# Antibas/eaQHM-analysis-and-synthesis-in-Python

Measured on AMD Instinct MI355X. Metric: analysis_frames_per_sec, higher is better.
Workload: dtype f64; 1 GPU; synth16k_60s_female_maxAdpt5; samples=960000, fs=16000, ls_frames_per_adaptation=63936, adaptations_executed=5, Kmax=59, track_bytes=906240000, parallelism=instants sharded x1 by LS cost; boundary records all-gathered per adaptation

## Files before the change

eaqhm-analysis-and-synthesis-in-python_amd/csrc/eaqhm_ls_common.h:

```cpp
#pragma once
#include "eaqhm_common.h"

namespace eaqhm {

#define PIVOT_TOL 2.5e-13

#define LS_NCLS 7
#define LS_BIG_CLASS (LS_NCLS - 1)

struct LsArgs {
  int mode;
  const double* s; long long L; double fs;
  const double* am_cur; const double* fm_cur; long long Lt; long long trk_t0; int Kmax;
  const int* frame_inst; const int* frame_c; const int* frame_wl; const double* frame_f0; const int* frame_K;
  const int* ncol; const int* cols; const unsigned char* seeded; const int* any_seed;
  int n_frames; int a_iter; double f0_stale; double f0min;
  double* records; double* raw_amp; double* raw_slope;
  double* scratch; size_t scratch_stride; int nmax; int Nmax; int Kcmax;
  int* work_counter;
  const unsigned short* zloc; const int* ztot; int zchunks;
  unsigned char* zflag;
  int* cls;
  unsigned long long* debug;
  int debug_diag;
// ... 85 lines not shown
  }
  __syncthreads();
  if (tid < 64) {
    double e = 0.0;
    for (int t = tid; t <= wl; t += 64) {
      const double sp = sig[mid + t], sm = sig[mid - t];
      e += W2[t] * ((t == 0) ? sp * sp : (sp * sp + sm * sm));
    }
#pragma unroll
    for (int o = 32; o > 0; o >>= 1) e += __shfl_xor(e, o);
    if (tid == 0) ssq[0] = e;
  }
  const int nm = 2 * n + 1;
  int NCH = 1;
  {
    int best = 0x7fffffff;
    for (int q = 1; q <= NCH_; ++q) {
      const int cost = ((nm * q + cthr - 1) / cthr) * ((wl + q - 1) / q + 4);
      if (cost < best) { best = cost; NCH = q; }
    }
  }
  const int CL = (wl + NCH - 1) / NCH;
  for (int task = tid; task < nm * NCH; task += nthr) {
    const int ch = task / nm, m = task - ch * nm;
    const int t0 = 1 + ch * CL, t1 = (t0 + CL - 1 < wl) ? (t0 + CL - 1) : wl;
    const double phi = (double)m * theta;
    double zr, zi, sr, si;
    sincos_cw((double)t0 * phi, &zi, &zr);
    sincos_cw(phi, &si, &sr);
    double a0 = 0, a1 = 0, a2 = 0, b0 = 0, b1 = 0, b2 = 0, b3 = 0;
    const bool rhs = m <= n;
    for (int t = t0; t <= t1; ++t) {
      if (t > t0 && ((t - t0) & 63) == 0) sincos_cw((double)t * phi, &zi, &zr);
      const double w2 = W2[t], tt = (double)t, w2t = w2 * tt;
      a0 = fma(w2, zr, a0);
      a1 = fma(w2t, zi, a1);
      a2 = fma(w2t * tt, zr, a2);
      if (rhs) {
        const double pa = PA[t], pb = PB[t];
        b0 = fma(pa, zr, b0);
        b1 = fma(pb, zi, b1);
        b2 = fma(tt * pb, zr, b2);
        b3 = fma(tt * pa, zi, b3);
      }
      const double nr = zr * sr - zi * si, ni = zr * si + zi * sr;
      zr = nr; zi = ni;
    }
    double* pp = part + (size_t)(ch * TZ_NQ) * TB + m;
    pp[0] = a0; pp[TB] = a1; pp[2 * TB] = a2;
    pp[3 * TB] = b0; pp[4 * TB] = b1; pp[5 * TB] = b2; pp[6 * TB] = b3;
  }
  __syncthreads();
  for (int q = tid; q < TZ_NQ * nm; q += nthr) {
    const int k = q / nm, m = q - k * nm;
    double v = 0.0;
    for (int ch = 0; ch < NCH; ++ch) v += part[(size_t)(ch * TZ_NQ + k) * TB + m];
    if (k < 3) v *= 2.0;
    if (k == 0) v += W2[0];
    if (k == 3 && m <= n) v += W2[0] * sig[mid];
    tab[k * TB + m] = v;
  }
  __syncthreads();
}

__device__ inline int toeplitz_harm(int c, int n) { return (c < n) ? -(c + 1) : (c - n); }
__device__ inline void toeplitz_gram(const double* tab, int TB, int p, int a, int b, int n, double& re, double& im) {
  const int m = toeplitz_harm(b, n) - toeplitz_harm(a, n), am = (m < 0) ? -m : m;
  re = 0.0; im = 0.0;
  if (p == 1) im = (m < 0) ? -tab[TB + am] : tab[TB + am];
  else re = tab[p * TB + am];
}
__device__ inline void toeplitz_rhs(const double* tab, int TB, int p, int b, int n, double& re, double& im) {
  const int h = toeplitz_harm(b, n), ah = (h < 0) ? -h : h;
  re = tab[(3 + 2 * p) * TB + ah];
  im = tab[(4 + 2 * p) * TB + ah];
  if (h < 0) im = -im;
}

#define XCOL(cc, el) (((cc) & ~15) | (((cc) + (el)) & 15))

template <int STRIDE, int NWAVES>
__device__ inline void prepare_slots(const LsArgs& A, double* Qf, double* Af, int Npad, double* ci,
                                     unsigned long long* masks, int* gappy, const int* mycols, int n, int N, int mid,
                                     int c, int wl, bool seeds, int lane, int wave, int nchs) {
  const double eps = 10e-5;
  const int nch = (N + 63) >> 6;
  const long long t0 = (long long)c - wl;
  const unsigned short* zloc = uni(A.zloc);
  const int* ztot = uni(A.ztot);
  const double* fm_all = uni(A.fm_cur);
  const double* am_all = uni(A.am_cur);
  const long long L = ((long long)uni((int)(A.Lt >> 32)) << 32) | (unsigned)uni((int)(A.Lt & 0xffffffffll));
  const int zchunks = uni(A.zchunks);
  const double w1 = uni(2.0 * M_PI / A.fs);
  auto centre = [&](int j, double fv, double av) {
    ci[j * STRIDE + STRIDE - 3] = 1.0 / (av + eps);
    double sn, cs;
    sincos_cw(fv * w1, &sn, &cs);
    ci[j * STRIDE + STRIDE - 2] = cs;
    ci[j * STRIDE + STRIDE - 1] = sn;
  };
  int anyg = 0;
  for (int j = threadIdx.x; j < n; j += blockDim.x) {
    const int k = mycols[j];
    const long long b = (long long)c + wl, a1 = (long long)c - wl - 1;
    const int cb = (int)(b >> 10), ca = (a1 >= 0) ? (int)(a1 >> 10) : 0;
    const double fmc = fm_all[(size_t)k * L + c], amc = am_all[(size_t)k * L + c];
    int zc = zloc[(size_t)k * L + b];
    for (int ch = ca; ch < cb; ++ch) zc += ztot[(size_t)k * zchunks + ch];
    if (a1 >= 0) zc -= zloc[(size_t)k * L + a1];
    const int g = (zc != 0 || (seeds && k == 0)) ? 1 : 0;
    gappy[j] = g;
    anyg |= g;
    ci[j * STRIDE + 0] = 0.0;
    ci[j * STRIDE + 1] = 0.0;
    const size_t trk = (size_t)k * L + t0;
    ((const double**)(ci + j * STRIDE))[2] = g ? (Qf + (size_t)j * Npad) : (fm_all + trk);
    ((const double**)(ci + j * STRIDE))[3] = g ? (Af + (size_t)j * Npad) : (am_all + trk);
    if (!g) centre(j, fmc, amc);
  }
  if (!__syncthreads_or(anyg)) return;
  for (int it = wave; it < n * nch; it += NWAVES) {
    const int j = it / nch, ch = it - j * nch, t = (ch << 6) + lane;
    if (!gappy[j]) continue;
    const double fv = (t < N) ? track_fm(A, mycols[j], t0 + t, c, seeds) : 0.0;
    const unsigned long long m = __ballot(fv != 0.0);
    if (lane == 0) masks[j * nchs + ch] = m;
  }
  __syncthreads();
  for (int it = wave; it < n * nch; it += NWAVES) {
    const int j = it / nch, ch = it - j * nch, t = (ch << 6) + lane, k = mycols[j];
    if (!gappy[j] || t >= N) continue;
    double fv = track_fm(A, k, t0 + t, c, seeds), av = track_am(A, k, t0 + t, c, seeds);
    if (fv == 0.0) {
      int p = -1, q = -1;
      {
        unsigned long long m = masks[j * nchs + ch] & ((lane == 0) ? 0ull : (~0ull >> (64 - lane)));
        int cc = ch;
        while (m == 0ull && cc > 0) { --cc; m = masks[j * nchs + cc]; }
        if (m != 0ull) p = (cc << 6) + 63 - __clzll((long long)m);
      }
      {
        unsigned long long m = masks[j * nchs + ch] & ((lane == 63) ? 0ull : (~0ull << (lane + 1)));
        int cc = ch;
        while (m == 0ull && cc < nch - 1) { ++cc; m = masks[j * nchs + cc]; }
        if (m != 0ull) q = (cc << 6) + __ffsll((long long)m) - 1;
      }
      if (p < 0) {
        fv = track_fm(A, k, t0 + q, c, seeds); av = track_am(A, k, t0 + q, c, seeds);
      } else if (q < 0) {
        fv = track_fm(A, k, t0 + p, c, seeds); av = track_am(A, k, t0 + p, c, seeds);
      } else {
        const double f0v = track_fm(A, k, t0 + p, c, seeds), f1v = track_fm(A, k, t0 + q, c, seeds);
        const double a0v = track_am(A, k, t0 + p, c, seeds), a1v = track_am(A, k, t0 + q, c, seeds);
        const double dx = (double)(q - p), xx = (double)(t - p);
        fv = ((f1v - f0v) / dx) * xx + f0v;
        av = ((a1v - a0v) / dx) * xx + a0v;
      }
    }
    Qf[(size_t)j * Npad + t] = fv;
    Af[(size_t)j * Npad + t] = av;
    if (t == mid) centre(j, fv, av);
  }
  __syncthreads();
}

template <int CTRL>
__device__ inline double dpp_row(double x) {
  const int lo = __builtin_amdgcn_update_dpp(0, __double2loint(x), CTRL, 0xf, 0xf, true);
  const int hi = __builtin_amdgcn_update_dpp(0, __double2hiint(x), CTRL, 0xf, 0xf, true);
  return __hiloint2double(hi, lo);
}
__device__ inline double scan16(double x) {
  x += dpp_row<0x111>(x);
  x += dpp_row<0x112>(x);
  x += dpp_row<0x114>(x);
  x += dpp_row<0x118>(x);
  return x;
}

__device__ inline void cholesky_solve(double* __restrict__ Lt, int M, int ldl, double* rowj, double* xs, double* sh,
                                      int* fault) {
  const int tid = threadIdx.x, nt = blockDim.x;
  for (int j = 0; j < M; ++j) {
    for (int k = tid; k < j; k += nt) {
      size_t o = ((size_t)k * ldl + j) * 2;
      rowj[2 * k] = Lt[o];
      rowj[2 * k + 1] = Lt[o + 1];
    }
    __syncthreads();
    for (int i = j + tid; i <= M; i += nt) {
      size_t oj = ((size_t)j * ldl + i) * 2;
      double ar = Lt[oj], ai = Lt[oj + 1];
      for (int k = 0; k < j; ++k) {
        size_t o = ((size_t)k * ldl + i) * 2;
        double lr = Lt[o], li = Lt[o + 1];
        double cr = rowj[2 * k], ci = rowj[2 * k + 1];
        ar -= lr * cr + li * ci;
        ai -= li * cr - lr * ci;
      }
      if (i == j) {
        if (!(ar > PIVOT_TOL * Lt[oj])) { atomicAdd(fault, 1); ar = 1.0; }
        double d = sqrt(ar);
        sh[0] = d;
        Lt[oj] = d; Lt[oj + 1] = 0.0;
      } else {
        Lt[oj] = ar; Lt[oj + 1] = ai;
      }
    }
    __syncthreads();
    double inv = 1.0 / sh[0];
    for (int i = j + 1 + tid; i <= M; i += nt) {
      size_t oj = ((size_t)j * ldl + i) * 2;
      Lt[oj] *= inv; Lt[oj + 1] *= inv;
    }
    __syncthreads();
  }
  if (tid < 64) {
    for (int j = M - 1; j >= 0; --j) {
      const double* row = Lt + (size_t)j * ldl * 2;
      double sr = 0, si = 0;
      for (int i = j + 1 + tid; i < M; i += 64) {
        double lr = row[2 * i], li = row[2 * i + 1];
        double xr = xs[2 * i], xi = xs[2 * i + 1];
        sr += lr * xr + li * xi;
        si += lr * xi - li * xr;
      }
      for (int o = 32; o > 0; o >>= 1) {
        sr += __shfl_xor(sr, o);
        si += __shfl_xor(si, o);
      }
      if (tid == 0) {
        double d = row[2 * j];
        double yr = row[2 * M], yi = -row[2 * M + 1];
        xs[2 * j] = (yr - sr) / d;
        xs[2 * j + 1] = (yi - si) / d;
      }
      __builtin_amdgcn_wave_barrier();
      __threadfence_block();
    }
  }
  __syncthreads();
}

__device__ inline void write_record(const LsArgs& A, const double* xs, double* sh, const int* mycols, int f, int n,
                                    int inst, int c, double f0, bool seeds) {
  const int tid = threadIdx.x, nt = blockDim.x, Kc = 2 * n + 1;
  if (A.raw_amp) {
    const int stride = 2 * (2 * A.Kmax + 1);
    for (int q = tid; q < 2 * Kc; q += nt) {
      const int col = q >> 1, src = (A.mode == 0 && col < n) ? (n - 1 - col) : col;
      A.raw_amp[(size_t)f * stride + q] = xs[2 * src + (q & 1)];
      A.raw_slope[(size_t)f * stride + q] = xs[2 * Kc + 2 * src + (q & 1)];
    }
  }
  double amax = 0.0;
  for (int j = tid; j < n; j += nt) {
    double ar = xs[2 * (n + 1 + j)], ai = xs[2 * (n + 1 + j) + 1];
    amax = fmax(amax, sqrt(ar * ar + ai * ai));
  }
  for (int o = 32; o > 0; o >>= 1) amax = fmax(amax, __shfl_xor(amax, o));
  if ((tid & 63) == 0) sh[1 + (tid >> 6)] = amax;
  __syncthreads();
  amax = 0.0;
  for (int w = 0; w < (nt >> 6); ++w) amax = fmax(amax, sh[1 + w]);
  const double floor_mag = amax * 3.1622776601683795e-08;
  const double h = f0 / (double)(A.a_iter + 1);
  double* rec = A.records + (size_t)inst * (3 * A.Kmax + 1);
  for (int k = tid; k < 3 * A.Kmax; k += nt) rec[k] = 0.0;
  __syncthreads();
  for (int j = tid; j < n; j += nt) {
    const int k = (A.mode == 0) ? j : mycols[j];
    double ar = xs[2 * (n + 1 + j)], ai = xs[2 * (n + 1 + j) + 1];
    double br = xs[2 * (Kc + n + 1 + j)], bi = xs[2 * (Kc + n + 1 + j) + 1];
    double mag = sqrt(ar * ar + ai * ai);
    double eta = 0.0;
    if (A.mode == 1) eta = A.fs / (2.0 * M_PI) * ((ar * bi - ai * br) / (mag * mag));
    if (mag > floor_mag && fabs(eta) < h) {
      rec[k] = mag;
      rec[2 * A.Kmax + k] = atan2(ai, ar);
      double fmv;
      if (A.mode == 0) fmv = (double)(k + 1) * f0;
      else {
        double cur = track_fm(A, k, c, c, seeds);
        fmv = (f0 > A.f0min) ? cur + eta : cur;
      }
      rec[A.Kmax + k] = fmv;
    }
  }
  if (tid == 0) rec[3 * A.Kmax] = xs[2 * n];
  __syncthreads();
}

}
```

eaqhm-analysis-and-synthesis-in-python_amd/csrc/eaqhm_ls_tile.hip:

```cpp
#include <type_traits>
#include "eaqhm_ls_common.h"
#include "eaqhm_ls_chol.h"
#include "eaqhm_ls_a0.h"
#include "eaqhm_ls_tilemap.h"
#include "eaqhm_ls_twunits.h"
#include "eaqhm_ls_gather.h"

namespace eaqhm {
bool ls_a0tile_fits(const LsArgs& A);
int launch_ls_a0tile(eaqhm_ctx* ctx, LsArgs A);

#define DIAG_OWNER(jb, nt) ((int)TL_DIAG[nt][jb])
#define TL_THREADS 512
#define TL_WAVES 8
#define TL_CW 8
#define TL_NTMAX 13
#define CI_STRIDE 20
#define CI_NCH 16

__device__ inline void tw_step(d4 (&g)[9], double aR, double aI, double bR, double bI, double nk) {
  const double sA = aR + aI, dB = bI - bR;
  const double naR = nk * aR, naI = nk * aI, nsA = nk * sA;
  const double nbR = nk * bR, nbI = nk * bI, ndB = nk * dB;
  g[0] = __builtin_amdgcn_mfma_f64_16x16x4f64(aR, bR, g[0], 0, 0, 0);
  g[1] = __builtin_amdgcn_mfma_f64_16x16x4f64(aI, bI, g[1], 0, 0, 0);
  g[2] = __builtin_amdgcn_mfma_f64_16x16x4f64(sA, dB, g[2], 0, 0, 0);
  g[3] = __builtin_amdgcn_mfma_f64_16x16x4f64(naR, bR, g[3], 0, 0, 0);
  g[4] = __builtin_amdgcn_mfma_f64_16x16x4f64(naI, bI, g[4], 0, 0, 0);
  g[5] = __builtin_amdgcn_mfma_f64_16x16x4f64(nsA, dB, g[5], 0, 0, 0);
  g[6] = __builtin_amdgcn_mfma_f64_16x16x4f64(naR, nbR, g[6], 0, 0, 0);
  g[7] = __builtin_amdgcn_mfma_f64_16x16x4f64(naI, nbI, g[7], 0, 0, 0);
  g[8] = __builtin_amdgcn_mfma_f64_16x16x4f64(nsA, ndB, g[8], 0, 0, 0);
}

__device__ inline void twu_pair_k3(d4 (&g0)[3], d4 (&g1)[3], d4 (&g2)[3], double aR, double aI, double bR, double bI, double nk) {
  const double sA = aR + aI, dB = bI - bR;
  const double naR = nk * aR, naI = nk * aI, nsA = nk * sA;
  const double nbR = nk * bR, nbI = nk * bI, ndB = nk * dB;
  g0[0] = __builtin_amdgcn_mfma_f64_16x16x4f64(aR, bR, g0[0], 0, 0, 0);
  g0[1] = __builtin_amdgcn_mfma_f64_16x16x4f64(aI, bI, g0[1], 0, 0, 0);
  g0[2] = __builtin_amdgcn_mfma_f64_16x16x4f64(sA, dB, g0[2], 0, 0, 0);
  g1[0] = __builtin_amdgcn_mfma_f64_16x16x4f64(naR, bR, g1[0], 0, 0, 0);
  g1[1] = __builtin_amdgcn_mfma_f64_16x16x4f64(naI, bI, g1[1], 0, 0, 0);
  g1[2] = __builtin_amdgcn_mfma_f64_16x16x4f64(nsA, dB, g1[2], 0, 0, 0);
  g2[0] = __builtin_amdgcn_mfma_f64_16x16x4f64(naR, nbR, g2[0], 0, 0, 0);
  g2[1] = __builtin_amdgcn_mfma_f64_16x16x4f64(naI, nbI, g2[1], 0, 0, 0);
  g2[2] = __builtin_amdgcn_mfma_f64_16x16x4f64(nsA, ndB, g2[2], 0, 0, 0);
}
__device__ inline void twu_pair_2acc(d4 (&g0)[2], d4 (&g1)[2], d4 (&g2)[2], double aR, double aI, double bR, double bI, double nk,
                                     bool k4) {
  const double naR = nk * aR, naI = nk * aI, nbR = nk * bR, nbI = nk * bI;
  g0[0] = __builtin_amdgcn_mfma_f64_16x16x4f64(aR, bR, g0[0], 0, 0, 0);
  g1[0] = __builtin_amdgcn_mfma_f64_16x16x4f64(naR, bR, g1[0], 0, 0, 0);
  g2[0] = __builtin_amdgcn_mfma_f64_16x16x4f64(naR, nbR, g2[0], 0, 0, 0);
  g0[1] = __builtin_amdgcn_mfma_f64_16x16x4f64(aR, bI, g0[1], 0, 0, 0);
  g1[1] = __builtin_amdgcn_mfma_f64_16x16x4f64(naR, bI, g1[1], 0, 0, 0);
  g2[1] = __builtin_amdgcn_mfma_f64_16x16x4f64(naR, nbI, g2[1], 0, 0, 0);
  g0[0] = __builtin_amdgcn_mfma_f64_16x16x4f64(aI, bI, g0[0], 0, 0, 0);
  g1[0] = __builtin_amdgcn_mfma_f64_16x16x4f64(naI, bI, g1[0], 0, 0, 0);
  g2[0] = __builtin_amdgcn_mfma_f64_16x16x4f64(naI, nbI, g2[0], 0, 0, 0);
  if (k4) {
    const double maI = -aI, mnaI = -naI;
    g0[1] = __builtin_amdgcn_mfma_f64_16x16x4f64(maI, bR, g0[1], 0, 0, 0);
    g1[1] = __builtin_amdgcn_mfma_f64_16x16x4f64(mnaI, bR, g1[1], 0, 0, 0);
    g2[1] = __builtin_amdgcn_mfma_f64_16x16x4f64(mnaI, nbR, g2[1], 0, 0, 0);
  }
}

__device__ inline void twu_edge_k4(d4 (&g0)[2], d4 (&g1)[2], double aR, double aI, double bR, double bI, double nk) {
  const double nbR = nk * bR, nbI = nk * bI, maI = -aI;
  g0[0] = __builtin_amdgcn_mfma_f64_16x16x4f64(aR, bR, g0[0], 0, 0, 0);
  g1[0] = __builtin_amdgcn_mfma_f64_16x16x4f64(aR, nbR, g1[0], 0, 0, 0);
  g0[1] = __builtin_amdgcn_mfma_f64_16x16x4f64(aR, bI, g0[1], 0, 0, 0);
  g1[1] = __builtin_amdgcn_mfma_f64_16x16x4f64(aR, nbI, g1[1], 0, 0, 0);
  g0[0] = __builtin_amdgcn_mfma_f64_16x16x4f64(aI, bI, g0[0], 0, 0, 0);
  g1[0] = __builtin_amdgcn_mfma_f64_16x16x4f64(aI, nbI, g1[0], 0, 0, 0);
  g0[1] = __builtin_amdgcn_mfma_f64_16x16x4f64(maI, bR, g0[1], 0, 0, 0);
  g1[1] = __builtin_amdgcn_mfma_f64_16x16x4f64(maI, nbR, g1[1], 0, 0, 0);
}

template <int NS, int TW, int UA = 0, int UB = 0, int TB = 0>
__device__ __attribute__((noinline)) void tile_frame(const LsArgs& A, int TS_, int ldx_max_, double* lds, int f_) {
  const int TS = uni(TS_), ldx_max = uni(ldx_max_), f = uni(f_);
  const int tid = threadIdx.x, nt_thr = TL_THREADS;
  const int lane = tid & 63;
  const int wave = __builtin_amdgcn_readfirstlane(tid >> 6);
  double* U = uni(lds);
  double* Xre = U;
  double* Xim = Xre + (size_t)TS * ldx_max;
  const size_t usize_g = (size_t)2 * TS * ldx_max;
  double* ci = U + usize_g;
  unsigned long long* masks = (unsigned long long*)(ci + (size_t)CI_STRIDE * 52);
  double* PanR = U;
  double* PanI = PanR + TL_NTMAX * TL_TILE;
  double* WtR = PanI + TL_NTMAX * TL_TILE;
  double* WtI = WtR + TL_NTMAX * TL_TILE;
  double* LdR = WtI + TL_NTMAX * TL_TILE;
  double* LdI = LdR + TL_TILE;
  double* Dc = LdI + TL_TILE;
  double* Zc = Dc + DG_TILE;
  double* zv = Zc + DG_TILE;
  double* xv = zv + 2 * 16 * TL_NTMAX;
  const size_t usize_c = (size_t)(xv + 32 - U);
  double* xs = U + usize_c;
  double* sh = xs + 4 * uni(A.Kcmax);
  double* win = sh + 16;
  double* sig = win + 64 * CI_NCH;
  double* dorig = sig + 64 * CI_NCH;

  const int Npad = ((uni(A.Nmax) + 63) >> 6) << 6;
  double* Qs = uni(A.scratch) + (size_t)blockIdx.x * (size_t)uni((int)A.scratch_stride);
  double* Rs = Qs + (size_t)Npad * uni(A.nmax);
  const bool seeds = uni((int)(A.any_seed && (*A.any_seed != 0))) != 0;
  const double w1 = uni(2.0 * M_PI / A.fs);
  const int PE = TS / 2;
  const double* sA = uni(A.s);
  const int lcol = lane & 15, lq = lane >> 4;
  unsigned long long* dbg = uni(A.debug);
  unsigned long long t_prev = 0;

  {
    const int n = uni(A.ncol[f]);
    const int Kc = 2 * n + 1, Ms = 2 * Kc + 1;
    const int nt = (Ms + 15) >> 4;
    const int c = uni(A.frame_c[f]), wl = uni(A.frame_wl[f]), inst = uni(A.frame_inst[f]);
    const int N = 2 * wl + 1, mid = wl;
    const int T = (Kc + 16) >> 4;
    constexpr int UN = UA + UB;
    constexpr int GA = UA / 3, GB = UB / 3;
    constexpr bool G3 = TW > 0 || UN > 0;
    static_assert(TW == 0 || UN == 0, "whole pairs or units");
    static_assert(UN == 0 || (UA == TWU_UA && UB == TWU_UB), "slot layout of eaqhm_ls_twunits.h");
    static_assert(TB >= 0 && TB < TWU_NTB, "unit table");
    constexpr bool PK = UN > 0 && TWU_PACKED[TB];
    constexpr int EC = 16 * (TWU_TT[TB] - 1);
    const int nb = G3 ? T : nt;
    const int ldx = (nb << 4) + ((nb & 1) ? 0 : 16);
    const int npair = T * (T + 1) / 2;
    const int is = 2 * Kc - 16 * (nt - 1);
    const double f0 = uni(A.f0_stale);
    const int* mycols = uni(A.cols) + (size_t)f * uni(A.Kmax);
    const int npairs = mid + 1;

    if (dbg && tid == 0) t_prev = __builtin_amdgcn_s_memtime();
    for (int q = tid; q < 2 * TS * ldx_max; q += nt_thr) Xre[q] = 0.0;
    for (int t = tid; t < N; t += nt_thr) {
      win[t] = window_value(false, t, N);
      sig[t] = sA[(size_t)(c - wl) + t];
    }
    __syncthreads();
    int* gappy = (int*)(masks + (size_t)52 * CI_NCH);
    prepare_slots<CI_STRIDE, TL_WAVES>(A, Qs, Rs, Npad, ci, masks, gappy, mycols, n, N, mid, c, wl, seeds, lane, wave, CI_NCH);
    LS_STAMP(0);

    constexpr int NM3 = (NS <= 7) ? NS : 0;
    d4 accR[NS], accI[NS], acc3[NM3 ? NM3 : 1];
    int tP[NS], tQ[NS];
    bool live[NS];
#pragma unroll
    for (int sl = 0; sl < NS; ++sl) {
      accR[sl] = (d4){0, 0, 0, 0};
      accI[sl] = (d4){0, 0, 0, 0};
      if (sl < NM3) acc3[sl] = (d4){0, 0, 0, 0};
      const int code = TL_MAP[nt][wave][sl];
      live[sl] = code != 0xFF;
      const int P = live[sl] ? (code >> 4) : 0, Q = live[sl] ? (code & 15) : 0;
      tP[sl] = __builtin_amdgcn_readfirstlane(P);
      tQ[sl] = __builtin_amdgcn_readfirstlane(Q);
    }

    constexpr int TWA = TW ? TW : 1;
    const bool split = TW > 0 && NS == 5 && T == 4;
    d4 g[TWA][9];
    int gI[TWA], gJ[TWA], gx[TWA];
    bool glive[TWA];
#pragma unroll
    for (int sl = 0; sl < TWA; ++sl) {
      const int x = (split && sl == 1) ? 8 + (wave >> 1) : wave + 8 * sl;
      glive[sl] = TW && x < npair && !(split && sl == 1 && wave >= 4);
      gx[sl] = __builtin_amdgcn_readfirstlane(x);
      int I = 0, J = 0;
      if (glive[sl]) tile_of(x, I, J);
      gI[sl] = __builtin_amdgcn_readfirstlane(I);
      gJ[sl] = __builtin_amdgcn_readfirstlane(J);
#pragma unroll
      for (int p = 0; p < 9; ++p) g[sl][p] = (d4){0, 0, 0, 0};
    }

    constexpr int UAA = UA > 3 ? UA : 3, UBA = UB > 3 ? UB : 3;
    d4 ga[UAA][3], gb[UBA][2];
    int ucode[UN ? UN : 1];
    if constexpr (UN > 0) {
#pragma unroll
      for (int sl = 0; sl < UN; ++sl) ucode[sl] = __builtin_amdgcn_readfirstlane((int)TWU_MAPS[TB][wave][sl]);
#pragma unroll
      for (int sl = 0; sl < UA; ++sl)
#pragma unroll
        for (int p = 0; p < 3; ++p) ga[sl][p] = (d4){0, 0, 0, 0};
#pragma unroll
      for (int sl = 0; sl < UB; ++sl) gb[sl][0] = gb[sl][1] = (d4){0, 0, 0, 0};
    }

    for (int d0 = 0; d0 < npairs; d0 += PE) {
#pragma clang loop unroll(disable)
      for (int idx = tid; idx < 16 * n; idx += nt_thr) {
        const int el = idx & 15, j = idx >> 4, d = d0 + el;
        const bool act = d <= mid;
        const int u = mid - d - 1, v = mid + d;
        double su = 0, cu = 1, sv, cv;
        double pur = 0, pui = 0, nur = 0, nui = 0, pvr, pvi, nvr, nvi;
        {
          double* cj = ci + j * CI_STRIDE;
          const double* fb = ((const double**)cj)[2];
          const double* ab = ((const double**)cj)[3];
          const int dc = act ? d : mid;
          const double fu1 = fb[mid - dc], fv = fb[mid + dc];
          const double au = ab[(mid - dc - 1 >= 0) ? (mid - dc - 1) : 0], au1 = ab[mid - dc];
          const double av = ab[mid + dc], av1 = ab[(mid + dc + 1 < N) ? (mid + dc + 1) : (N - 1)];
          const double xu = act ? fu1 : 0.0, xv = (act && d >= 1) ? fv : 0.0;
          const double qv = cj[0] + scan16(xv), qu = -(cj[1] + scan16(xu));
          if (el == 15) { cj[0] = qv; cj[1] = -qu; }
          if (!act) continue;
          const double ainv = cj[17], pr = cj[18], pi = cj[19];
          sincos_cw(qu * w1, &su, &cu);
          sincos_cw(qv * w1, &sv, &cv);
          const double eps = 10e-5;
          if (u >= 0) {
            const double ru = (eps + au) * ainv, rv1 = (eps + av1) * ainv;
            pur = ru * cu;                    pui = ru * su;
            nur = rv1 * (cv * pr - sv * pi);  nui = rv1 * (cv * pi + sv * pr);
          }
          const double rv = (eps + av) * ainv, ru1 = (eps + au1) * ainv;
          pvr = rv * cv;                      pvi = rv * sv;
          nvr = ru1 * (cu * pr - su * pi);    nvi = ru1 * (cu * pi + su * pr);
        }
// ... 359 lines not shown
      }
      LS_STAMP(uni((int)A.debug_diag) ? 2 : 9);
    }

    {
#pragma unroll
      for (int sl = 0; sl < NS; ++sl) {
        if (!live[sl] || tP[sl] != nt - 1) continue;
#pragma unroll
        for (int r = 0; r < 4; ++r) {
          const int row = lq + 4 * r, col = lcol;
          const bool pad = (row > is) || (tQ[sl] == nt - 1 && col > is);
          if (pad) {
            accR[sl][r] = (tQ[sl] == nt - 1 && row == col) ? 1.0 : 0.0;
            accI[sl][r] = 0.0;
          }
        }
      }
#pragma unroll
      for (int sl = 0; sl < NS; ++sl) {
        if (!live[sl] || tP[sl] != tQ[sl]) continue;
#pragma unroll
        for (int r = 0; r < 4; ++r)
          if (lq + 4 * r == lcol) dorig[16 * tP[sl] + lcol] = accR[sl][r];
      }
      double* post = Dc;
      double* dumpD = Dc + DGP_DOUBLES;
      double* zs = dumpD + 128;
      int* dflag = (int*)(zs + 256);
      if (tid == 0) *dflag = 0;
      __syncthreads();
#define TRAILING_UPDATE(sl)                                                                         \
  {                                                                                                 \
    const double* ar = PanR + tP[sl] * TL_TILE;                                                     \
    const double* ai = PanI + tP[sl] * TL_TILE;                                                     \
    const double* br = PanR + tQ[sl] * TL_TILE;                                                     \
    const double* bi = PanI + tQ[sl] * TL_TILE;                                                     \
       \
       \
    d4 p1 = (d4){0, 0, 0, 0}, p2 = (d4){0, 0, 0, 0};                                                \
    _Pragma("unroll") for (int ks = 0; ks < 4; ++ks) {                                              \
      const int o = (4 * ks + lq) * TL_LD + lcol;                                                   \
      const double aR = ar[o], aI = ai[o], lR = br[o], lI = bi[o];                                  \
      p1 = __builtin_amdgcn_mfma_f64_16x16x4f64(aR, lR, p1, 0, 0, 0);                               \
      p2 = __builtin_amdgcn_mfma_f64_16x16x4f64(aI, lI, p2, 0, 0, 0);                               \
      accI[sl] = __builtin_amdgcn_mfma_f64_16x16x4f64(aR + aI, lI - lR, accI[sl], 0, 0, 0);         \
    }                                                                                               \
    accR[sl] = accR[sl] - (p1 + p2);                                                                \
    accI[sl] = accI[sl] + (p1 - p2);                                                                \
  }
      for (int jb = 0; jb < nt; ++jb) {
        d4 Rt = (d4){0, 0, 0, 0}, It = (d4){0, 0, 0, 0};
        bool mine = false;
#pragma unroll
        for (int sl = 0; sl < NS; ++sl) {
          if (!live[sl] || tP[sl] != jb || tQ[sl] != jb) continue;
          if (jb > 0) TRAILING_UPDATE(sl)
          Rt = accR[sl]; It = accI[sl];
          mine = true;
        }
        if (mine) {
          unsigned long long td0 = 0;
          unsigned long long* tlast = (unsigned long long*)(dflag + 2);
          const bool tdiag = dbg && uni(A.debug_diag);
          if (tdiag) td0 = __builtin_amdgcn_s_memtime();
          diag_D(Rt, It, post, nullptr, dflag, 16 * jb, dumpD, LdR, LdI, jb == nt - 1);
          if (tdiag && lane == 0) {
            const unsigned long long td1 = __builtin_amdgcn_s_memtime();
            atomicAdd(dbg + 9, td1 - td0);
            if (jb > 0) { atomicAdd(dbg + 11, td0 - *tlast); atomicAdd(dbg + 14, 1ull); }
            atomicAdd(dbg + 13, 1ull);
            *tlast = td1;
          }
        }
        LS_STAMP(10);
        if (jb > 0) {
#pragma unroll
          for (int sl = 0; sl < NS; ++sl) {
            if (!live[sl] || tQ[sl] < jb || (tP[sl] == jb && tQ[sl] == jb)) continue;
            TRAILING_UPDATE(sl)
          }
        }
        LS_STAMP(8);
        if (!mine && wave == (int)TL_HELP[nt][jb])
          diag_Z(post, dflag, 16 * jb, zs, WtR + jb * TL_TILE, WtI + jb * TL_TILE, dorig + 16 * jb,
                 (jb == nt - 1) ? is : 16, uni(A.fault));
        __syncthreads();
        LS_STAMP(6);
#pragma unroll
        for (int sl = 0; sl < NS; ++sl) {
          if (!live[sl] || tQ[sl] != jb || tP[sl] == jb) continue;
          double* tr = PanR + tP[sl] * TL_TILE;
          double* ti = PanI + tP[sl] * TL_TILE;
#pragma unroll
          for (int r = 0; r < 4; ++r) {
            tr[lcol * TL_LD + lq + 4 * r] = accR[sl][r];
            ti[lcol * TL_LD + lq + 4 * r] = accI[sl][r];
          }
          __builtin_amdgcn_wave_barrier();
          d4 p1 = (d4){0, 0, 0, 0}, p2 = (d4){0, 0, 0, 0}, p3 = (d4){0, 0, 0, 0};
          const double* wr = WtR + jb * TL_TILE;
          const double* wi = WtI + jb * TL_TILE;
#pragma unroll
          for (int ks = 0; ks < 4; ++ks) {
            const int o = (4 * ks + lq) * TL_LD + lcol;
            const double aR = tr[o], aI = ti[o], bR = wr[o], bI = wi[o];
            p1 = __builtin_amdgcn_mfma_f64_16x16x4f64(aR, bR, p1, 0, 0, 0);
            p2 = __builtin_amdgcn_mfma_f64_16x16x4f64(aI, bI, p2, 0, 0, 0);
            p3 = __builtin_amdgcn_mfma_f64_16x16x4f64(aR + aI, bR + bI, p3, 0, 0, 0);
          }
          const d4 xr = p1 - p2, xi = p3 - (p1 + p2);
          accR[sl] = xr; accI[sl] = xi;
          __builtin_amdgcn_wave_barrier();
#pragma unroll
          for (int r = 0; r < 4; ++r) {
            tr[lcol * TL_LD + lq + 4 * r] = xr[r];
            ti[lcol * TL_LD + lq + 4 * r] = xi[r];
          }
        }
        LS_STAMP(7);
        __syncthreads();
      }
#undef TRAILING_UPDATE
      __syncthreads();
      LS_STAMP(3);

#pragma unroll
      for (int sl = 0; sl < NS; ++sl) {
        if (!live[sl] || tP[sl] != nt - 1 || tQ[sl] == nt - 1) continue;
        if (lq == (is & 3)) {
#pragma unroll
          for (int r = 0; r < 4; ++r)
            if (r == (is >> 2)) {
              zv[2 * (16 * tQ[sl] + lcol)] = accR[sl][r];
              zv[2 * (16 * tQ[sl] + lcol) + 1] = -accI[sl][r];
            }
        }
      }
      if (tid < 16) {
        const bool ok = tid < is;
        zv[2 * (16 * (nt - 1) + tid)] = ok ? LdR[is * TL_LD + tid] : 0.0;
        zv[2 * (16 * (nt - 1) + tid) + 1] = ok ? -LdI[is * TL_LD + tid] : 0.0;
      }
      for (int q = tid; q < 4 * Kc; q += nt_thr) xs[q] = 0.0;
      __syncthreads();
      for (int P = nt - 1; P >= 0; --P) {
        if (tid < 256) {
          const int i = tid >> 4, k = tid & 15;
          double xr = 0, xi = 0;
          if (k >= i) {
            const double wr = WtR[P * TL_TILE + i * TL_LD + k], wi = WtI[P * TL_TILE + i * TL_LD + k];
            const double zr = zv[2 * (16 * P + k)], zi = zv[2 * (16 * P + k) + 1];
            xr = wr * zr - wi * zi;
            xi = wr * zi + wi * zr;
          }
#pragma unroll
          for (int o = 8; o > 0; o >>= 1) { xr += __shfl_xor(xr, o); xi += __shfl_xor(xi, o); }
          if (k == 0) {
            xv[2 * i] = xr; xv[2 * i + 1] = xi;
            const int q = 16 * P + i;
            if (q < 2 * Kc) { xs[2 * q] = xr; xs[2 * q + 1] = xi; }
          }
        }
        __syncthreads();
#pragma unroll
        for (int sl = 0; sl < NS; ++sl) {
          if (!live[sl] || tP[sl] != P || tQ[sl] == P) continue;
          double sr = 0, si = 0;
#pragma unroll
          for (int r = 0; r < 4; ++r) {
            const double xr = xv[2 * (lq + 4 * r)], xi = xv[2 * (lq + 4 * r) + 1];
            const double lr = accR[sl][r], li = accI[sl][r];
            sr += lr * xr + li * xi;
            si += lr * xi - li * xr;
          }
          sr += __shfl_xor(sr, 16); si += __shfl_xor(si, 16);
          sr += __shfl_xor(sr, 32); si += __shfl_xor(si, 32);
          if (lq == 0) {
            zv[2 * (16 * tQ[sl] + lcol)] -= sr;
            zv[2 * (16 * tQ[sl] + lcol) + 1] -= si;
          }
        }
        __syncthreads();
      }
      LS_STAMP(4);
    }

    write_record(A, xs, sh, mycols, f, n, inst, c, f0, seeds);
    LS_STAMP(5);
  }
}

__device__ inline int frame_class(int n) {
  const int nt = (2 * (2 * n + 1) + 1 + 15) >> 4;
  return nt <= 8 ? 0 : nt == 9 ? 1 : nt == 10 ? 2 : nt == 11 ? 3 : nt == 12 ? 4 : nt <= TL_NTMAX ? 5 : LS_BIG_CLASS;
}
extern "C" __global__ void __launch_bounds__(256) eaqhm_ls_classify_kernel(LsArgs A) {
  const int f = blockIdx.x * blockDim.x + threadIdx.x, lane = threadIdx.x & 63;
  int cl = (f < A.n_frames) ? frame_class((A.mode == 0) ? A.frame_K[f] : A.ncol[f]) : -1;
  if (f < A.n_frames) {
    if (!frame_window_ok(A, A.frame_c[f], A.frame_wl[f])) { cl = -1; atomicAdd(A.fault + 2, 1); }
  }
  if (A.mode == 1 && cl >= 0) {
    const long long c = A.frame_c[f], wl = A.frame_wl[f];
    const long long lo = (c - wl - 1 > 0) ? (c - wl - 1) : 0;
    for (long long ch = lo >> 10; ch <= ((c + wl) >> 10); ++ch) A.zflag[ch] = 1;
  }
  for (int c = 0; c < LS_NCLS; ++c) {
    const unsigned long long m = __ballot(cl == c);
    if (m == 0ull) continue;
    int base = 0;
    if (lane == __ffsll((long long)m) - 1) base = atomicAdd(A.cls + c, __popcll(m));
    base = __shfl(base, __ffsll((long long)m) - 1);
    if (cl == c) A.cls[16 + (size_t)c * A.n_frames + base + __popcll(m & ((1ull << lane) - 1ull))] = f;
  }
}

extern "C" __global__ void __launch_bounds__(256) eaqhm_ls_zero_prefix_kernel(const double* __restrict__ fm, long long Lt,
                                                                              long long t_lo, int ch0, int zchunks,
                                                                              const unsigned char* __restrict__ zflag,
                                                                              unsigned short* __restrict__ zloc,
                                                                              int* __restrict__ ztot) {
  __shared__ int wsum[4];
  const int k = blockIdx.y, ch = ch0 + blockIdx.x, tid = threadIdx.x, lane = tid & 63, wave = tid >> 6;
  if (!zflag[ch]) return;
  const long long base = (long long)ch << 10;
  int run = 0;
  for (int p = 0; p < 4; ++p) {
    const long long t = base + 256 * p + tid;
    const bool in = t >= t_lo && t < t_lo + Lt;
    const bool z = in && (fm[(size_t)k * Lt + t] == 0.0);
    const unsigned long long m = __ballot(z);
    const int incl = __popcll(m & ((lane == 63) ? ~0ull : ((1ull << (lane + 1)) - 1ull)));
    if (lane == 0) wsum[wave] = __popcll(m);
    __syncthreads();
    int off = 0, tot = 0;
#pragma unroll
    for (int w = 0; w < 4; ++w) { const int v = wsum[w]; tot += v; if (w < wave) off += v; }
    if (in) zloc[(size_t)k * Lt + t] = (unsigned short)(run + off + incl);
    run += tot;
    __syncthreads();
  }
  if (tid == 0) ztot[(size_t)k * zchunks + ch] = run;
}

extern "C" __global__ void __launch_bounds__(TL_THREADS) eaqhm_ls_tile_kernel(LsArgs A, int TS, int ldx_max) {
  extern __shared__ __attribute__((aligned(16))) double lds[];
  __shared__ int nxt;
#define TW_UNITS(TB) 0, TWU_UA, TWU_UB, TB
#define RUN_CLASS(NSV, TWV, C)                                                             \
  for (;;) {                                                                             \
    if (threadIdx.x == 0) nxt = atomicAdd(A.cls + 8 + C, 1);                             \
    __syncthreads();                                                                     \
    const int item = nxt;                                                                \
    __syncthreads();                                                                     \
    if (item >= A.cls[C]) break;                                                         \
    if (A.mode == 0) a0_frame<A0_NS, A0_M, 2>(A, lds, A.cls[16 + (size_t)C * A.n_frames + item], TZ_TB, TZ_NCH, 520, 64 * CI_NCH);                          \
    else tile_frame<NSV, TWV>(A, TS, ldx_max, lds, A.cls[16 + (size_t)C * A.n_frames + item]);          \
  }
  RUN_CLASS(12, 0, 5)
  RUN_CLASS(10, TW_UNITS(TWU_TB_12), 4)
  RUN_CLASS(9, TW_UNITS(TWU_TB_11), 3)
  RUN_CLASS(7, 2, 2)
  RUN_CLASS(6, 2, 1)
  RUN_CLASS(5, 2, 0)
#undef RUN_CLASS
#undef TW_UNITS
}

#define TL_LDS_LIMIT (159 * 1024)
static size_t tl_usize_c() {
  return (size_t)4 * TL_NTMAX * TL_TILE + 2 * TL_TILE + 2 * DG_TILE + 2 * 16 * TL_NTMAX + 32;
}
static size_t tl_usize_g(int TS, int ldx_max) { return (size_t)2 * TS * ldx_max + (size_t)CI_STRIDE * 52 + 52 * CI_NCH + 32; }
static size_t tl_lds_doubles(int Kcmax, int TS, int ldx_max) {
  const size_t c = tl_usize_c(), g = tl_usize_g(TS, ldx_max);
  return (c > g ? c : g) + 4 * (size_t)Kcmax + 16 + 2 * 64 * CI_NCH + 16 * TL_NTMAX;
}

bool ls_tile_applicable(int Kcmax, int Nmax) {
  return Nmax <= 64 * CI_NCH && tl_lds_doubles(Kcmax, 32, 16 * TL_NTMAX + 16) * sizeof(double) <= TL_LDS_LIMIT;
}

size_t ls_tile_scratch_stride(int nmax, int Nmax) {
  const size_t Npad = (size_t)((Nmax + 63) >> 6) << 6;
  const size_t bridged = 2 * Npad * nmax, gram = (size_t)3 * 21 * 512 + 2;
  return ((bridged > gram ? bridged : gram) + 15) & ~(size_t)15;
}

int launch_ls_prepass(eaqhm_ctx* ctx, LsArgs A, long long track_t0) {
  hipLaunchKernelGGL(eaqhm_ls_classify_kernel, dim3((A.n_frames + 255) / 256), dim3(256), 0, ctx->stream, A);
  HIP_TRY(ctx, hipGetLastError());
  if (A.mode == 1) {
    const int ch0 = (int)(track_t0 >> 10), ch1 = (int)((track_t0 + A.Lt - 1) >> 10);
    hipLaunchKernelGGL(eaqhm_ls_zero_prefix_kernel, dim3(ch1 - ch0 + 1, A.Kmax), dim3(256), 0, ctx->stream, A.fm_cur, A.Lt,
                       track_t0, ch0, A.zchunks, A.zflag, (unsigned short*)A.zloc, (int*)A.ztot);
    HIP_TRY(ctx, hipGetLastError());
  }
  return EAQHM_OK;
}

int launch_ls_tile(eaqhm_ctx* ctx, LsArgs A, int grid) {
  if (A.mode == 0 && ctx->a0_resident && ls_a0tile_fits(A)) return launch_ls_a0tile(ctx, A);
  const int Kcmax = A.Kcmax;
  const int ldx_max = 16 * TL_NTMAX + 16;
  const int TS = 32;
  const size_t lds_bytes = tl_lds_doubles(Kcmax, TS, ldx_max) * sizeof(double);
  if (lds_bytes > TL_LDS_LIMIT) return ctx->fail(EAQHM_EINVAL, "eaqhm_ls_batch: LDS budget exceeded (tile variant)");
  if (a0_lds_doubles(A0_M, 2, TZ_TB, TZ_NCH, 520, 64 * CI_NCH, Kcmax) * sizeof(double) > lds_bytes)
    return ctx->fail(EAQHM_EINVAL, "eaqhm_ls_batch: LDS budget exceeded (adaptation 0, tile variant)");
  HIP_TRY(ctx, hipFuncSetAttribute((const void*)eaqhm_ls_tile_kernel, hipFuncAttributeMaxDynamicSharedMemorySize, (int)lds_bytes));
  hipLaunchKernelGGL(eaqhm_ls_tile_kernel, dim3(grid), dim3(TL_THREADS), lds_bytes, ctx->stream, A, TS, ldx_max);
  HIP_TRY(ctx, hipGetLastError());
  return EAQHM_OK;
}

}
```

Before: 1.659 million frames/s.

## Prefetch next frame header during solve and stage records in LDS

Adds a persistent LDS header so one idle wave fetches the next work item (atomic, frame params, column list) during the Cholesky phase, removing the serialized atomic plus barriers between frames. Also replaces shuffle reductions with DPP/permlane-swap reductions, overlaps signal loads with zeroing of the X tiles, and for the NS=9 class builds the output record in LDS with a cached centre frequency before copying it out contiguously. This adds LDS layout constraints, more control complexity and a new header region whose placement must not overlap other buffers.

```diff
diff --git a/eaqhm-analysis-and-synthesis-in-python_amd/csrc/eaqhm_ls_common.h b/eaqhm-analysis-and-synthesis-in-python_amd/csrc/eaqhm_ls_common.h
--- a/eaqhm-analysis-and-synthesis-in-python_amd/csrc/eaqhm_ls_common.h
+++ b/eaqhm-analysis-and-synthesis-in-python_amd/csrc/eaqhm_ls_common.h
@@ -191,7 +191,7 @@
 template <int STRIDE, int NWAVES>
 __device__ inline void prepare_slots(const LsArgs& A, double* Qf, double* Af, int Npad, double* ci,
                                      unsigned long long* masks, int* gappy, const int* mycols, int n, int N, int mid,
-                                     int c, int wl, bool seeds, int lane, int wave, int nchs) {
+                                     int c, int wl, bool seeds, int lane, int wave, int nchs, double* fstash = nullptr) {
   const double eps = 10e-5;
   const int nch = (N + 63) >> 6;
   const long long t0 = (long long)c - wl;
@@ -227,6 +227,7 @@
     ((const double**)(ci + j * STRIDE))[2] = g ? (Qf + (size_t)j * Npad) : (fm_all + trk);
     ((const double**)(ci + j * STRIDE))[3] = g ? (Af + (size_t)j * Npad) : (am_all + trk);
     if (!g) centre(j, fmc, amc);
+    if (fstash) fstash[j] = g ? -1.0 : fmc;
   }
   if (!__syncthreads_or(anyg)) return;
   for (int it = wave; it < n * nch; it += NWAVES) {
@@ -287,6 +288,32 @@
   x += dpp_row<0x118>(x);
   return x;
 }
+__device__ inline double sum16_first(double x) {
+  x += dpp_row<0x108>(x);
+  x += dpp_row<0x104>(x);
+  x += dpp_row<0x102>(x);
+  x += dpp_row<0x101>(x);
+  return x;
+}
+__device__ inline double sum4rows_first(double x) {
+  {
+    const auto lo = __builtin_amdgcn_permlane16_swap(__double2loint(x), __double2loint(x), false, false);
+    const auto hi = __builtin_amdgcn_permlane16_swap(__double2hiint(x), __double2hiint(x), false, false);
+    x = __hiloint2double(hi[0], lo[0]) + __hiloint2double(hi[1], lo[1]);
+  }
+  const auto lo = __builtin_amdgcn_permlane32_swap(__double2loint(x), __double2loint(x), false, false);
+  const auto hi = __builtin_amdgcn_permlane32_swap(__double2hiint(x), __double2hiint(x), false, false);
+  return __hiloint2double(hi[0], lo[0]) + __hiloint2double(hi[1], lo[1]);
+}
+__device__ inline double max64_nonneg_last(double x) {
+  x = fmax(x, dpp_row<0x111>(x));
+  x = fmax(x, dpp_row<0x112>(x));
+  x = fmax(x, dpp_row<0x114>(x));
+  x = fmax(x, dpp_row<0x118>(x));
+  x = fmax(x, dpp_row<0x142>(x));
+  x = fmax(x, dpp_row<0x143>(x));
+  return x;
+}
 
 __device__ inline void cholesky_solve(double* __restrict__ Lt, int M, int ldl, double* rowj, double* xs, double* sh,
                                       int* fault) {
@@ -352,8 +379,10 @@
   __syncthreads();
 }
 
+template <bool ROW = false>
 __device__ inline void write_record(const LsArgs& A, const double* xs, double* sh, const int* mycols, int f, int n,
-                                    int inst, int c, double f0, bool seeds) {
+                                    int inst, int c, double f0, bool seeds, const double* fstash = nullptr,
+                                    double* row = nullptr) {
   const int tid = threadIdx.x, nt = blockDim.x, Kc = 2 * n + 1;
   if (A.raw_amp) {
     const int stride = 2 * (2 * A.Kmax + 1);
@@ -368,16 +397,25 @@
     double ar = xs[2 * (n + 1 + j)], ai = xs[2 * (n + 1 + j) + 1];
     amax = fmax(amax, sqrt(ar * ar + ai * ai));
   }
-  for (int o = 32; o > 0; o >>= 1) amax = fmax(amax, __shfl_xor(amax, o));
-  if ((tid & 63) == 0) sh[1 + (tid >> 6)] = amax;
+  if constexpr (ROW) {
+    amax = max64_nonneg_last(amax);
+    if ((tid & 63) == 63) sh[1 + (tid >> 6)] = amax;
+    for (int k = tid; k < 3 * A.Kmax; k += nt) row[k] = 0.0;
+  } else {
+    for (int o = 32; o > 0; o >>= 1) amax = fmax(amax, __shfl_xor(amax, o));
+    if ((tid & 63) == 0) sh[1 + (tid >> 6)] = amax;
+  }
   __syncthreads();
   amax = 0.0;
   for (int w = 0; w < (nt >> 6); ++w) amax = fmax(amax, sh[1 + w]);
   const double floor_mag = amax * 3.1622776601683795e-08;
   const double h = f0 / (double)(A.a_iter + 1);
   double* rec = A.records + (size_t)inst * (3 * A.Kmax + 1);
-  for (int k = tid; k < 3 * A.Kmax; k += nt) rec[k] = 0.0;
-  __syncthreads();
+  double* dst = ROW ? row : rec;
+  if constexpr (!ROW) {
+    for (int k = tid; k < 3 * A.Kmax; k += nt) rec[k] = 0.0;
+    __syncthreads();
+  }
   for (int j = tid; j < n; j += nt) {
     const int k = (A.mode == 0) ? j : mycols[j];
     double ar = xs[2 * (n + 1 + j)], ai = xs[2 * (n + 1 + j) + 1];
@@ -386,19 +424,21 @@
     double eta = 0.0;
     if (A.mode == 1) eta = A.fs / (2.0 * M_PI) * ((ar * bi - ai * br) / (mag * mag));
     if (mag > floor_mag && fabs(eta) < h) {
-      rec[k] = mag;
-      rec[2 * A.Kmax + k] = atan2(ai, ar);
+      dst[k] = mag;
+      dst[2 * A.Kmax + k] = atan2(ai, ar);
       double fmv;
       if (A.mode == 0) fmv = (double)(k + 1) * f0;
       else {
-        double cur = track_fm(A, k, c, c, seeds);
+        double cur = (ROW && fstash[j] >= 0.0) ? fstash[j] : track_fm(A, k, c, c, seeds);
         fmv = (f0 > A.f0min) ? cur + eta : cur;
       }
-      rec[A.Kmax + k] = fmv;
-    }
-  }
-  if (tid == 0) rec[3 * A.Kmax] = xs[2 * n];
-  __syncthreads();
-}
-
-}
+      dst[A.Kmax + k] = fmv;
+    }
+  }
+  if (tid == 0) dst[3 * A.Kmax] = xs[2 * n];
+  __syncthreads();
+  if constexpr (ROW)
+    for (int k = tid; k <= 3 * A.Kmax; k += nt) rec[k] = row[k];
+}
+
+}
diff --git a/eaqhm-analysis-and-synthesis-in-python_amd/csrc/eaqhm_ls_tile.hip b/eaqhm-analysis-and-synthesis-in-python_amd/csrc/eaqhm_ls_tile.hip
--- a/eaqhm-analysis-and-synthesis-in-python_amd/csrc/eaqhm_ls_tile.hip
+++ b/eaqhm-analysis-and-synthesis-in-python_amd/csrc/eaqhm_ls_tile.hip
@@ -5,6 +5,7 @@
 #include "eaqhm_ls_tilemap.h"
 #include "eaqhm_ls_twunits.h"
 #include "eaqhm_ls_gather.h"
+#include "eaqhm_ls_tilelds.h"
 
 namespace eaqhm {
 bool ls_a0tile_fits(const LsArgs& A);
@@ -14,9 +15,23 @@
 #define TL_THREADS 512
 #define TL_WAVES 8
 #define TL_CW 8
-#define TL_NTMAX 13
-#define CI_STRIDE 20
-#define CI_NCH 16
+static_assert(TLL_TILE == TL_TILE && TLL_DG_TILE == DG_TILE, "eaqhm_ls_tilelds.h and eaqhm_ls_chol.h disagree");
+
+__device__ inline void fetch_next_header(const LsArgs& A, TlHead* hd, int C, int nbuf, int lane) {
+  int* cls = uni(A.cls);
+  int item = 0;
+  if (lane == 0) item = atomicAdd(cls + 8 + C, 1);
+  item = uni(item);
+  int f = -1;
+  if (item < uni(cls[C])) f = uni(cls[16 + (size_t)C * uni(A.n_frames) + item]);
+  if (f >= 0) {
+    const int* tab = (lane == 0) ? A.ncol : (lane == 1) ? A.frame_c : (lane == 2) ? A.frame_wl : A.frame_inst;
+    if (lane < 4) (&hd->n)[lane] = tab[f];
+    const int Kmax = uni(A.Kmax);
+    if (lane < TL_NSLOT && lane < Kmax) hd->cols[nbuf][lane] = A.cols[(size_t)f * Kmax + lane];
+  }
+  if (lane == 0) { hd->f = f; hd->buf = nbuf; hd->cls = C; }
+}
 
 __device__ inline void tw_step(d4 (&g)[9], double aR, double aI, double bR, double bI, double nk) {
   const double sA = aR + aI, dB = bI - bR;
@@ -81,11 +96,17 @@
 
 template <int NS, int TW, int UA = 0, int UB = 0, int TB = 0>
 __device__ __attribute__((noinline)) void tile_frame(const LsArgs& A, int TS_, int ldx_max_, double* lds, int f_) {
-  const int TS = uni(TS_), ldx_max = uni(ldx_max_), f = uni(f_);
+  constexpr int C = NS == 12 ? 5 : NS == 10 ? 4 : NS == 9 ? 3 : NS == 7 ? 2 : NS == 6 ? 1 : 0;
+  static_assert(NS == 12 || NS == 10 || NS == 9 || NS == 7 || NS == 6 || NS == 5, "a register budget per class");
+  constexpr bool NEXT_HEAD = NS != 10, REC_ROW = NS == 9;
+  const bool pre = uni(f_) < 0;
+  const int TS = uni(TS_), ldx_max = uni(ldx_max_);
   const int tid = threadIdx.x, nt_thr = TL_THREADS;
   const int lane = tid & 63;
   const int wave = __builtin_amdgcn_readfirstlane(tid >> 6);
   double* U = uni(lds);
+  TlHead* hd = (TlHead*)(U + tl_head_offset());
+  const int f = pre ? uni(hd->f) : uni(f_);
   double* Xre = U;
   double* Xim = Xre + (size_t)TS * ldx_max;
   const size_t usize_g = (size_t)2 * TS * ldx_max;
@@ -101,8 +122,7 @@
   double* Zc = Dc + DG_TILE;
   double* zv = Zc + DG_TILE;
   double* xv = zv + 2 * 16 * TL_NTMAX;
-  const size_t usize_c = (size_t)(xv + 32 - U);
-  double* xs = U + usize_c;
+  double* xs = xv + 32 + TL_HEAD_DOUBLES;
   double* sh = xs + 4 * uni(A.Kcmax);
   double* win = sh + 16;
   double* sig = win + 64 * CI_NCH;
@@ -111,7 +131,7 @@
   const int Npad = ((uni(A.Nmax) + 63) >> 6) << 6;
   double* Qs = uni(A.scratch) + (size_t)blockIdx.x * (size_t)uni((int)A.scratch_stride);
   double* Rs = Qs + (size_t)Npad * uni(A.nmax);
-  const bool seeds = uni((int)(A.any_seed && (*A.any_seed != 0))) != 0;
+  const bool seeds = uni(hd->seeds) != 0;
   const double w1 = uni(2.0 * M_PI / A.fs);
   const int PE = TS / 2;
   const double* sA = uni(A.s);
@@ -120,10 +140,11 @@
   unsigned long long t_prev = 0;
 
   {
-    const int n = uni(A.ncol[f]);
+    const int n = pre ? uni(hd->n) : uni(A.ncol[f]);
     const int Kc = 2 * n + 1, Ms = 2 * Kc + 1;
     const int nt = (Ms + 15) >> 4;
-    const int c = uni(A.frame_c[f]), wl = uni(A.frame_wl[f]), inst = uni(A.frame_inst[f]);
+    const int c = pre ? uni(hd->c) : uni(A.frame_c[f]), wl = pre ? uni(hd->wl) : uni(A.frame_wl[f]);
+    const int inst = pre ? uni(hd->inst) : uni(A.frame_inst[f]);
     const int N = 2 * wl + 1, mid = wl;
     const int T = (Kc + 16) >> 4;
     constexpr int UN = UA + UB;
@@ -139,18 +160,28 @@
     const int npair = T * (T + 1) / 2;
     const int is = 2 * Kc - 16 * (nt - 1);
     const double f0 = uni(A.f0_stale);
-    const int* mycols = uni(A.cols) + (size_t)f * uni(A.Kmax);
+    const int* mycols = pre ? (const int*)hd->cols[uni(hd->buf)] : uni(A.cols) + (size_t)f * uni(A.Kmax);
     const int npairs = mid + 1;
 
-    if (dbg && tid == 0) t_prev = __builtin_amdgcn_s_memtime();
-    for (int q = tid; q < 2 * TS * ldx_max; q += nt_thr) Xre[q] = 0.0;
-    for (int t = tid; t < N; t += nt_thr) {
-      win[t] = window_value(false, t, N);
-      sig[t] = sA[(size_t)(c - wl) + t];
+    if (dbg && tid == 0) {
+      t_prev = __builtin_amdgcn_s_memtime();
+      if (hd->t_last && !uni((int)A.debug_diag)) atomicAdd(dbg + 11, t_prev - hd->t_last);
     }
-    __syncthreads();
+    double sv[2];
+#pragma unroll
+    for (int r = 0; r < 2; ++r) {
+      const int t = tid + r * nt_thr;
+      sv[r] = (t < N) ? sA[(size_t)(c - wl) + t] : 0.0;
+    }
+    for (int q = tid; q < TS * ldx; q += nt_thr) { Xre[q] = 0.0; Xim[q] = 0.0; }
+#pragma unroll
+    for (int r = 0; r < 2; ++r) {
+      const int t = tid + r * nt_thr;
+      if (t < N) { win[t] = window_value(false, t, N); sig[t] = sv[r]; }
+    }
     int* gappy = (int*)(masks + (size_t)52 * CI_NCH);
-    prepare_slots<CI_STRIDE, TL_WAVES>(A, Qs, Rs, Npad, ci, masks, gappy, mycols, n, N, mid, c, wl, seeds, lane, wave, CI_NCH);
+    prepare_slots<CI_STRIDE, TL_WAVES>(A, Qs, Rs, Npad, ci, masks, gappy, mycols, n, N, mid, c, wl, seeds, lane, wave, CI_NCH,
+                                       REC_ROW ? hd->fmc : nullptr);
     LS_STAMP(0);
 
     constexpr int NM3 = (NS <= 7) ? NS : 0;
@@ -676,6 +707,11 @@
           }
         }
         LS_STAMP(8);
+        if (NEXT_HEAD && jb == 0) {
+          int pfw = 0;
+          while (pfw == DIAG_OWNER(0, nt) || pfw == (int)TL_HELP[nt][0]) ++pfw;
+          if (wave == pfw) fetch_next_header(A, hd, C, uni(hd->buf) ^ 1, lane);
+        }
         if (!mine && wave == (int)TL_HELP[nt][jb])
           diag_Z(post, dflag, 16 * jb, zs, WtR + jb * TL_TILE, WtI + jb * TL_TILE, dorig + 16 * jb,
                  (jb == nt - 1) ? is : 16, uni(A.fault));
@@ -748,8 +784,7 @@
             xr = wr * zr - wi * zi;
             xi = wr * zi + wi * zr;
           }
-#pragma unroll
-          for (int o = 8; o > 0; o >>= 1) { xr += __shfl_xor(xr, o); xi += __shfl_xor(xi, o); }
+          xr = sum16_first(xr); xi = sum16_first(xi);
           if (k == 0) {
             xv[2 * i] = xr; xv[2 * i + 1] = xi;
             const int q = 16 * P + i;
@@ -768,8 +803,7 @@
             sr += lr * xr + li * xi;
             si += lr * xi - li * xr;
           }
-          sr += __shfl_xor(sr, 16); si += __shfl_xor(si, 16);
-          sr += __shfl_xor(sr, 32); si += __shfl_xor(si, 32);
+          sr = sum4rows_first(sr); si = sum4rows_first(si);
           if (lq == 0) {
             zv[2 * (16 * tQ[sl] + lcol)] -= sr;
             zv[2 * (16 * tQ[sl] + lcol) + 1] -= si;
@@ -780,8 +814,12 @@
       LS_STAMP(4);
     }
 
-    write_record(A, xs, sh, mycols, f, n, inst, c, f0, seeds);
+    if (REC_ROW && 3 * uni(A.Kmax) + 1 <= TL_NSLOT * CI_NCH)
+      write_record<true>(A, xs, sh, mycols, f, n, inst, c, f0, seeds, hd->fmc, (double*)masks);
+    else
+      write_record(A, xs, sh, mycols, f, n, inst, c, f0, seeds);
     LS_STAMP(5);
+    if (dbg && tid == 0) hd->t_last = t_prev;
   }
 }
 
@@ -841,10 +879,18 @@
 extern "C" __global__ void __launch_bounds__(TL_THREADS) eaqhm_ls_tile_kernel(LsArgs A, int TS, int ldx_max) {
   extern __shared__ __attribute__((aligned(16))) double lds[];
   __shared__ int nxt;
+  TlHead* hd = (TlHead*)(lds + tl_head_offset());
+  if (threadIdx.x == 0 && A.mode != 0) { hd->cls = -1; hd->t_last = 0ull; hd->seeds = (A.any_seed && *A.any_seed != 0) ? 1 : 0; }
+  __syncthreads();
 #define TW_UNITS(TB) 0, TWU_UA, TWU_UB, TB
 #define RUN_CLASS(NSV, TWV, C)                                                             \
   for (;;) {                                                                             \
-    if (threadIdx.x == 0) nxt = atomicAdd(A.cls + 8 + C, 1);                             \
+    if (A.mode != 0 && hd->cls == C) {                                                   \
+      if (hd->f < 0) break;                                                              \
+      tile_frame<NSV, TWV>(A, TS, ldx_max, lds, -1);                                     \
+      continue;                                                                          \
+    }                                                                                    \
+    if (threadIdx.x == 0) { nxt = atomicAdd(A.cls + 8 + C, 1); if (A.mode != 0) hd->buf = 1; }   \
     __syncthreads();                                                                     \
     const int item = nxt;                                                                \
     __syncthreads();                                                                     \
@@ -862,19 +908,7 @@
 #undef TW_UNITS
 }
 
-#define TL_LDS_LIMIT (159 * 1024)
-static size_t tl_usize_c() {
-  return (size_t)4 * TL_NTMAX * TL_TILE + 2 * TL_TILE + 2 * DG_TILE + 2 * 16 * TL_NTMAX + 32;
-}
-static size_t tl_usize_g(int TS, int ldx_max) { return (size_t)2 * TS * ldx_max + (size_t)CI_STRIDE * 52 + 52 * CI_NCH + 32; }
-static size_t tl_lds_doubles(int Kcmax, int TS, int ldx_max) {
-  const size_t c = tl_usize_c(), g = tl_usize_g(TS, ldx_max);
-  return (c > g ? c : g) + 4 * (size_t)Kcmax + 16 + 2 * 64 * CI_NCH + 16 * TL_NTMAX;
-}
-
-bool ls_tile_applicable(int Kcmax, int Nmax) {
-  return Nmax <= 64 * CI_NCH && tl_lds_doubles(Kcmax, 32, 16 * TL_NTMAX + 16) * sizeof(double) <= TL_LDS_LIMIT;
-}
+bool ls_tile_applicable(int Kcmax, int Nmax) { return tl_applicable(Kcmax, Nmax); }
 
 size_t ls_tile_scratch_stride(int nmax, int Nmax) {
   const size_t Npad = (size_t)((Nmax + 63) >> 6) << 6;
@@ -901,6 +935,7 @@
   const int TS = 32;
   const size_t lds_bytes = tl_lds_doubles(Kcmax, TS, ldx_max) * sizeof(double);
   if (lds_bytes > TL_LDS_LIMIT) return ctx->fail(EAQHM_EINVAL, "eaqhm_ls_batch: LDS budget exceeded (tile variant)");
+  if (!tl_layout_ok(TS, ldx_max)) return ctx->fail(EAQHM_EINVAL, "eaqhm_ls_batch: LDS layout (tile variant)");
   if (a0_lds_doubles(A0_M, 2, TZ_TB, TZ_NCH, 520, 64 * CI_NCH, Kcmax) * sizeof(double) > lds_bytes)
     return ctx->fail(EAQHM_EINVAL, "eaqhm_ls_batch: LDS budget exceeded (adaptation 0, tile variant)");
   HIP_TRY(ctx, hipFuncSetAttribute((const void*)eaqhm_ls_tile_kernel, hipFuncAttributeMaxDynamicSharedMemorySize, (int)lds_bytes));
diff --git a/eaqhm-analysis-and-synthesis-in-python_amd/csrc/eaqhm_ls_tilelds.h b/eaqhm-analysis-and-synthesis-in-python_amd/csrc/eaqhm_ls_tilelds.h
--- /dev/null
+++ b/eaqhm-analysis-and-synthesis-in-python_amd/csrc/eaqhm_ls_tilelds.h
@@ -0,0 +1,45 @@
+#pragma once
+#include <cstddef>
+
+#if defined(__HIPCC__)
+#define TLL_HD __host__ __device__
+#else
+#define TLL_HD
+#endif
+
+#define TL_NTMAX 13
+#define CI_STRIDE 20
+#define CI_NCH 16
+#define TL_NSLOT 52
+#define TLL_TILE (16 * 17)
+#define TLL_DG_TILE (2 * 16 * 17)
+#define TL_LDS_LIMIT (159 * 1024)
+
+#define TL_HEAD_GAP 16
+struct TlHead {
+  double gap[TL_HEAD_GAP];
+  double fmc[TL_NSLOT];
+  unsigned long long t_last;
+  int cls, f, n, c, wl, inst, buf, seeds;
+  int cols[2][TL_NSLOT];
+  int even[2];
+};
+static_assert(sizeof(TlHead) % 16 == 0, "TlHead: a multiple of 16 bytes");
+#define TL_HEAD_DOUBLES ((sizeof(TlHead) + 7) / 8)
+
+TLL_HD inline size_t tl_usize_c() {
+  return (size_t)4 * TL_NTMAX * TLL_TILE + 2 * TLL_TILE + 2 * TLL_DG_TILE + 2 * 16 * TL_NTMAX + 32;
+}
+TLL_HD inline size_t tl_usize_g(int TS, int ldx_max) {
+  return (size_t)2 * TS * ldx_max + (size_t)CI_STRIDE * TL_NSLOT + TL_NSLOT * CI_NCH + 32;
+}
+TLL_HD inline size_t tl_head_offset() { return tl_usize_c(); }
+TLL_HD inline bool tl_layout_ok(int TS, int ldx_max) { return tl_usize_g(TS, ldx_max) <= tl_usize_c() + TL_HEAD_GAP; }
+TLL_HD inline size_t tl_lds_doubles(int Kcmax, int TS, int ldx_max) {
+  const size_t c = tl_usize_c() + TL_HEAD_DOUBLES, g = tl_usize_g(TS, ldx_max);
+  return (c > g ? c : g) + 4 * (size_t)Kcmax + 16 + 2 * 64 * CI_NCH + 16 * TL_NTMAX;
+}
+
+inline bool tl_applicable(int Kcmax, int Nmax) {
+  return Nmax <= 64 * CI_NCH && tl_layout_ok(32, 16 * TL_NTMAX + 16) && tl_lds_doubles(Kcmax, 32, 16 * TL_NTMAX + 16) * sizeof(double) <= TL_LDS_LIMIT;
+}
```

Result: faster. 1.692 million frames/s (median of 6 runs) (+2.0%).
